# FastLM/CXL-SpecKV

Hardware: AMD Instinct MI355X
Metric: KV blocks/s fetch+decompress (higher is better)
Workload: dtype fp32 (int8 records -> fp16)

## Files before the change

cxl-speckv_amd/csrc/attend_kv.hip:

```cpp
#include "kernels.hpp"
#include "attend_fp8_device.hpp"

namespace speckv {

template <bool WINDOW>
__global__ __launch_bounds__(256) __attribute__((amdgpu_waves_per_eu(4, 4))) void k_attend_k8v4(AttendArgs a, const AttendKvSide* __restrict__ vside)
{
    const uint32_t lane = threadIdx.x & 63u;
    const uint32_t wave = __builtin_amdgcn_readfirstlane(threadIdx.x >> 6);
    const uint32_t c = lane & 15u, kb = lane >> 4;
    const uint32_t split = a.rows_first ? blockIdx.y : blockIdx.x, by = a.rows_first ? blockIdx.x : blockIdx.y;
    if (a.rows_first && by >= a.rows_real) return;
    const uint32_t hq = a.heads / 4u;
    uint32_t seq = by / hq;
    if (a.order) seq = a.order[seq];
    const uint32_t head = (by % hq) * 4u + wave;
    const uint64_t row = static_cast<uint64_t>(seq) * a.heads + head;
    const AttendSeq sq = a.seqs[seq];
    if (split >= sq.n_splits) {
        if (sq.n_splits == 0u && split == 0u) attend_zero_rows(a.direct_out, a.direct_lse, a.g, row, lane);
        return;
    }
    const AttendKvSide vsd = vside[seq];
    const uint64_t part = sq.part_base + static_cast<uint64_t>(head) * sq.n_splits + split;
    const uint32_t n_pages = sq.n_pages;
    const uint32_t skip_pos = WINDOW ? a.seq_skip[seq] : 0u;

    uint32_t qd[8];
    float qscale = 1.0f;
    auto quantise_query = [&]() { fp8_query_operand(a.q16 + (row * a.g + min(c, a.g - 1u)) * 128u + kb * 16u, c < a.g, a.scale_log2e, qd, qscale); };

    const uint32_t n_tiles = (n_pages + 15u) / 16u;
    const uint32_t t0 = split * sq.tiles_per_split;
    const uint32_t t1 = min(t0 + sq.tiles_per_split, n_tiles);
    float m_run = -INFINITY, l_run = 0.0f;
    f32x4 acc[8];
#pragma unroll
    for (int t = 0; t < 8; ++t) acc[t] = f32x4{0.0f, 0.0f, 0.0f, 0.0f};

    if (t0 < t1) {
        const uint8_t* kp = sq.lin_base + sq.k_first * 2048ull + head * 128u + kb * 16u + (static_cast<uint64_t>(t0) * 32u + c) * 1024u;
        const float* kt = sq.scale_tab + (sq.k_first + static_cast<uint64_t>(t0) * 16u) + 4u * kb;
        const uint8_t* vtile = vsd.v_base + ((vsd.v_first >> 4) + t0) * static_cast<uint64_t>(kMx4TileBytes);
        const uint8_t* vp = vtile + 2u * kb * 1024u + head * 128u + 8u * c;
        const uint8_t* vc = vtile + kMx4CodePlane + 2u * kb * 64u + head * 8u + (c >> 1);

        uint4 kx[2][2];
        uint2 vx[4];
        uint32_t vcode[4];
        f32x4 ks4;
        auto issue_k = [&]() {
#pragma unroll
            for (int b = 0; b < 2; ++b) { kx[b][0] = ldg16(kp + 16384 * b); kx[b][1] = ldg16(kp + 16384 * b + 64); }
            ks4 = ldg_f4(kt);
        };
        auto issue_v = [&]() {
#pragma unroll
            for (int r = 0; r < 4; ++r) vx[r] = ldg8(vp + 1024 * (r & 1) + 8192 * (r >> 1));
#pragma unroll
            for (int r = 0; r < 4; ++r) vcode[r] = ldg1(vc + 64 * (r & 1) + 512 * (r >> 1));
        };
        __builtin_amdgcn_sched_barrier(0);
        issue_k();
        __builtin_amdgcn_sched_barrier(0);
        issue_v();
        __builtin_amdgcn_sched_barrier(0);
        quantise_query();
        __builtin_amdgcn_sched_barrier(0);
        const bool ragged = (n_pages & 15u) != 0u;
#pragma unroll 1
        for (uint32_t tile = t0; tile < t1; ++tile) {
            const uint32_t step = (tile + 1u < t1) ? 1u : 0u;
            float sc[8];
#pragma unroll
            for (int b = 0; b < 2; ++b) fp8_scores(kx[b][0], kx[b][1], qd, ks4, qscale, b, sc);
            if (ragged && tile + 1u == n_tiles) {
#pragma unroll
                for (int r = 0; r < 4; ++r) {
                    const uint32_t pg = tile * 16u + att_slot_page(kb, r);
                    if (pg >= n_pages) { sc[2 * r] = -INFINITY; sc[2 * r + 1] = -INFINITY; vcode[r] = 0u; }
                }
            }
            if (WINDOW && tile == 0u && skip_pos != 0u) {
#pragma unroll
                for (int r = 0; r < 4; ++r) {
                    const uint32_t pg = att_slot_page(kb, r);
                    if (2u * pg < skip_pos) sc[2 * r] = -INFINITY;
                    if (2u * pg + 1u < skip_pos) sc[2 * r + 1] = -INFINITY;
                    if (2u * pg + 2u <= skip_pos) vcode[r] = 0u;
                }
            }
            __builtin_amdgcn_sched_barrier(0);
            kp += step * 32768u; kt += step * 16u;
            issue_k();
            __builtin_amdgcn_sched_barrier(0);
            float m_use;
            const float f = att_softmax_step(sc, m_run, m_use);
            float psum = 0.0f;
            f16x8 P;
#pragma unroll
            for (int j = 0; j < 8; ++j) {
                const float p = __builtin_amdgcn_exp2f(sc[j] - m_use);
                psum += p;
                P[j] = static_cast<_Float16>(p);
            }
            l_run = l_run * f + psum;
            float vsc[4];
#pragma unroll
            for (int r = 0; r < 4; ++r) vsc[r] = __uint_as_float(vcode[r] << 23);
#define KV_PV(T, WORD, SEL)                                                                                                       \
    {                                                                                                                              \
        const u32x4 vw = {__builtin_bit_cast(uint32_t, __builtin_amdgcn_cvt_scalef32_pk_f16_fp4(vx[0].WORD, vsc[0], SEL)),          \
                          __builtin_bit_cast(uint32_t, __builtin_amdgcn_cvt_scalef32_pk_f16_fp4(vx[1].WORD, vsc[1], SEL)),          \
                          __builtin_bit_cast(uint32_t, __builtin_amdgcn_cvt_scalef32_pk_f16_fp4(vx[2].WORD, vsc[2], SEL)),          \
                          __builtin_bit_cast(uint32_t, __builtin_amdgcn_cvt_scalef32_pk_f16_fp4(vx[3].WORD, vsc[3], SEL))};         \
        acc[T] = __builtin_amdgcn_mfma_f32_16x16x32_f16(__builtin_bit_cast(f16x8, vw), P, acc[T] * f, 0, 0, 0);                     \
    }
            KV_PV(0, x, 0) KV_PV(1, x, 1) KV_PV(2, x, 2) KV_PV(3, x, 3) KV_PV(4, y, 0) KV_PV(5, y, 1) KV_PV(6, y, 2) KV_PV(7, y, 3)
#undef KV_PV
            __builtin_amdgcn_sched_barrier(0);
            vp += step * kMx4TileBytes; vc += step * kMx4TileBytes;
            issue_v();
            __builtin_amdgcn_sched_barrier(0);
        }
    }
    att_store_rows8(a, acc, m_run, l_run, 1.0f, sq.n_splits == 1u, row, part, c, kb);
}

hipError_t launch_attend_k8v4(const AttendArgs& a, const AttendKvSide* d_vside, uint32_t n_seq, bool merge, float* d_out, float* d_lse, hipStream_t s)
{
    if (n_seq == 0) return hipSuccess;
    if (!a.seqs || !d_vside || !a.q16 || a.direct_out != d_out || a.heads % 4u || a.g == 0 || a.g > 16u) return hipErrorInvalidValue;
    AttendArgs ar = a;
    const uint32_t rows = n_seq * (a.heads / 4u), splits = a.n_splits ? a.n_splits : 1u;
    ar.rows_real = rows;
    const dim3 gr = a.rows_first ? dim3(rows | 1u, splits) : dim3(splits, rows);
    if (a.seq_skip) hipLaunchKernelGGL(k_attend_k8v4<true>, gr, dim3(256), 0, s, ar, d_vside);
    else hipLaunchKernelGGL(k_attend_k8v4<false>, gr, dim3(256), 0, s, ar, d_vside);
    const hipError_t e = hipGetLastError();
    if (e != hipSuccess || !merge) return e;
    return launch_attend_combine(a, n_seq, d_out, d_lse, s);
}

}
```

Baseline: 772.9 million.

## Double-buffer V tile loads two tiles ahead in the k8v4 attend kernel

Splits the V operand registers into two alternating sets (vA/vB) and unrolls the tile loop by two, so each tile's V loads are issued two iterations ahead instead of one. This gives the V fetches more time to arrive before the PV MFMAs use them and hides memory latency. The cost is more live VGPRs under a fixed waves-per-EU bound of 4, which could cause spills. The scale codes are also narrowed to uint8 storage.

```diff
diff --git a/cxl-speckv_amd/csrc/attend_kv.hip b/cxl-speckv_amd/csrc/attend_kv.hip
--- a/cxl-speckv_amd/csrc/attend_kv.hip
+++ b/cxl-speckv_amd/csrc/attend_kv.hip
@@ -45,32 +45,25 @@
         const uint8_t* vp = vtile + 2u * kb * 1024u + head * 128u + 8u * c;
         const uint8_t* vc = vtile + kMx4CodePlane + 2u * kb * 64u + head * 8u + (c >> 1);
 
+        struct VSet { uint2 x[4]; uint8_t code[4]; };
         uint4 kx[2][2];
-        uint2 vx[4];
-        uint32_t vcode[4];
         f32x4 ks4;
-        auto issue_k = [&]() {
+        VSet vA, vB;
+        auto issue_k = [&](uint32_t step) __attribute__((always_inline)) {
+            kp += step * 32768u; kt += step * 16u;
 #pragma unroll
             for (int b = 0; b < 2; ++b) { kx[b][0] = ldg16(kp + 16384 * b); kx[b][1] = ldg16(kp + 16384 * b + 64); }
             ks4 = ldg_f4(kt);
         };
-        auto issue_v = [&]() {
+        auto issue_v = [&](VSet& v, uint32_t step) __attribute__((always_inline)) {
+            vp += step * kMx4TileBytes; vc += step * kMx4TileBytes;
 #pragma unroll
-            for (int r = 0; r < 4; ++r) vx[r] = ldg8(vp + 1024 * (r & 1) + 8192 * (r >> 1));
+            for (int r = 0; r < 4; ++r) v.x[r] = ldg8(vp + 1024 * (r & 1) + 8192 * (r >> 1));
 #pragma unroll
-            for (int r = 0; r < 4; ++r) vcode[r] = ldg1(vc + 64 * (r & 1) + 512 * (r >> 1));
+            for (int r = 0; r < 4; ++r) v.code[r] = static_cast<uint8_t>(ldg1(vc + 64 * (r & 1) + 512 * (r >> 1)));
         };
-        __builtin_amdgcn_sched_barrier(0);
-        issue_k();
-        __builtin_amdgcn_sched_barrier(0);
-        issue_v();
-        __builtin_amdgcn_sched_barrier(0);
-        quantise_query();
-        __builtin_amdgcn_sched_barrier(0);
         const bool ragged = (n_pages & 15u) != 0u;
-#pragma unroll 1
-        for (uint32_t tile = t0; tile < t1; ++tile) {
-            const uint32_t step = (tile + 1u < t1) ? 1u : 0u;
+        auto do_tile = [&](uint32_t tile, VSet& v) __attribute__((always_inline)) {
             float sc[8];
 #pragma unroll
             for (int b = 0; b < 2; ++b) fp8_scores(kx[b][0], kx[b][1], qd, ks4, qscale, b, sc);
@@ -78,7 +71,7 @@
 #pragma unroll
                 for (int r = 0; r < 4; ++r) {
                     const uint32_t pg = tile * 16u + att_slot_page(kb, r);
-                    if (pg >= n_pages) { sc[2 * r] = -INFINITY; sc[2 * r + 1] = -INFINITY; vcode[r] = 0u; }
+                    if (pg >= n_pages) { sc[2 * r] = -INFINITY; sc[2 * r + 1] = -INFINITY; v.code[r] = 0u; }
                 }
             }
             if (WINDOW && tile == 0u && skip_pos != 0u) {
@@ -87,12 +80,11 @@
                     const uint32_t pg = att_slot_page(kb, r);
                     if (2u * pg < skip_pos) sc[2 * r] = -INFINITY;
                     if (2u * pg + 1u < skip_pos) sc[2 * r + 1] = -INFINITY;
-                    if (2u * pg + 2u <= skip_pos) vcode[r] = 0u;
+                    if (2u * pg + 2u <= skip_pos) v.code[r] = 0u;
                 }
             }
             __builtin_amdgcn_sched_barrier(0);
-            kp += step * 32768u; kt += step * 16u;
-            issue_k();
+            issue_k((tile + 1u < t1) ? 1u : 0u);
             __builtin_amdgcn_sched_barrier(0);
             float m_use;
             const float f = att_softmax_step(sc, m_run, m_use);
@@ -107,22 +99,37 @@
             l_run = l_run * f + psum;
             float vsc[4];
 #pragma unroll
-            for (int r = 0; r < 4; ++r) vsc[r] = __uint_as_float(vcode[r] << 23);
+            for (int r = 0; r < 4; ++r) vsc[r] = __uint_as_float(static_cast<uint32_t>(v.code[r]) << 23);
 #define KV_PV(T, WORD, SEL)                                                                                                       \
     {                                                                                                                              \
-        const u32x4 vw = {__builtin_bit_cast(uint32_t, __builtin_amdgcn_cvt_scalef32_pk_f16_fp4(vx[0].WORD, vsc[0], SEL)),          \
-                          __builtin_bit_cast(uint32_t, __builtin_amdgcn_cvt_scalef32_pk_f16_fp4(vx[1].WORD, vsc[1], SEL)),          \
-                          __builtin_bit_cast(uint32_t, __builtin_amdgcn_cvt_scalef32_pk_f16_fp4(vx[2].WORD, vsc[2], SEL)),          \
-                          __builtin_bit_cast(uint32_t, __builtin_amdgcn_cvt_scalef32_pk_f16_fp4(vx[3].WORD, vsc[3], SEL))};         \
+        const u32x4 vw = {__builtin_bit_cast(uint32_t, __builtin_amdgcn_cvt_scalef32_pk_f16_fp4(v.x[0].WORD, vsc[0], SEL)),         \
+                          __builtin_bit_cast(uint32_t, __builtin_amdgcn_cvt_scalef32_pk_f16_fp4(v.x[1].WORD, vsc[1], SEL)),         \
+                          __builtin_bit_cast(uint32_t, __builtin_amdgcn_cvt_scalef32_pk_f16_fp4(v.x[2].WORD, vsc[2], SEL)),         \
+                          __builtin_bit_cast(uint32_t, __builtin_amdgcn_cvt_scalef32_pk_f16_fp4(v.x[3].WORD, vsc[3], SEL))};        \
         acc[T] = __builtin_amdgcn_mfma_f32_16x16x32_f16(__builtin_bit_cast(f16x8, vw), P, acc[T] * f, 0, 0, 0);                     \
     }
             KV_PV(0, x, 0) KV_PV(1, x, 1) KV_PV(2, x, 2) KV_PV(3, x, 3) KV_PV(4, y, 0) KV_PV(5, y, 1) KV_PV(6, y, 2) KV_PV(7, y, 3)
 #undef KV_PV
             __builtin_amdgcn_sched_barrier(0);
-            vp += step * kMx4TileBytes; vc += step * kMx4TileBytes;
-            issue_v();
+            issue_v(v, (tile + 2u < t1) ? 1u : 0u);
             __builtin_amdgcn_sched_barrier(0);
+        };
+        __builtin_amdgcn_sched_barrier(0);
+        issue_k(0u);
+        __builtin_amdgcn_sched_barrier(0);
+        issue_v(vA, 0u);
+        __builtin_amdgcn_sched_barrier(0);
+        issue_v(vB, (t0 + 1u < t1) ? 1u : 0u);
+        __builtin_amdgcn_sched_barrier(0);
+        quantise_query();
+        __builtin_amdgcn_sched_barrier(0);
+        uint32_t tile = t0;
+#pragma unroll 1
+        for (; tile + 1u < t1; tile += 2u) {
+            do_tile(tile, vA);
+            do_tile(tile + 1u, vB);
         }
+        if (tile < t1) do_tile(tile, vA);
     }
     att_store_rows8(a, acc, m_run, l_run, 1.0f, sq.n_splits == 1u, row, part, c, kb);
 }
```

Result: no change. 772.8 million (median of 4 runs) (-0.0%).
